# gk969/stm32-speech-recognition

Hardware: AMD Instinct MI355X
Metric: utterances/sec (256-frame, 100 templates) (higher is better)
Workload: dtype int32

## Files before the change

### stm32_speech_recognition_amd/csrc/k_mfcc.hip

```cpp
#include "sr_fft_dev.h"

#include <type_traits>

#ifndef SR_MEL_CHUNKED
#define SR_MEL_CHUNKED 1
#endif

namespace sr {

constexpr int kMfccWaves = 4;
constexpr int kFramesPerWave = 16, kFramesPerWaveMid = 4, kFramesPerWaveSmall = 1;
#ifndef SR_MAG_TAB_BINS
#define SR_MAG_TAB_BINS 8
#endif
constexpr int mfcc_tab_bins(int fpw) { return fpw == kFramesPerWave ? SR_MAG_TAB_BINS : 0; }
static_assert(SR_MAG_TAB_BINS == 0 || SR_MAG_TAB_BINS == 4 || SR_MAG_TAB_BINS == 8, "table bins per lane");
#ifndef SR_MFCC_PIPE
#define SR_MFCC_PIPE 1
#endif
#ifndef SR_MFCC_PIPE_PEEL
#define SR_MFCC_PIPE_PEEL 1
#endif
#ifndef SR_MFCC_PIPE_VMCNT
#define SR_MFCC_PIPE_VMCNT (SR_MFCC_PIPE_PEEL ? 3 : 0)
#endif
static_assert(SR_MFCC_PIPE_VMCNT == 0 || (SR_MFCC_PIPE_VMCNT == 3 && SR_MFCC_PIPE_PEEL), "younger loads counted by the wait");
constexpr bool mfcc_pipelined(int fpw) { return SR_MFCC_PIPE && mfcc_tab_bins(fpw) == 8; }
#ifndef SR_MFCC_TM_REGS
#define SR_MFCC_TM_REGS 1
#endif
#ifdef SR_INJECT_LDS_RACE
#undef SR_MFCC_TM_REGS
#define SR_MFCC_TM_REGS 0
#endif
constexpr bool mfcc_tm_regs(int fpw) { return SR_MFCC_TM_REGS && mfcc_pipelined(fpw); }
constexpr int kMelPad = kMel + 1;
__device__ __forceinline__ constexpr int mel_chunk_word(int j) { return 256 * ((j >> 2) & 1) + 4 * ((j >> 3) ^ (4 * ((j >> 2) & 1))) + (j & 3); }
#ifndef SR_MFCC_PREFIX_TID
#define SR_MFCC_PREFIX_TID 1
#endif
__device__ __forceinline__ constexpr int mel_prefix_word(int j)
{
#if SR_MFCC_PREFIX_TID
    return 64 * (j & 7) + (j >> 3);
#elif SR_MEL_CHUNKED
    return mel_chunk_word(j);
#else
    return j;
#endif
}
#pragma clang diagnostic push
#pragma clang diagnostic ignored "-Winline-asm"
__device__ __forceinline__ void mel_prefix_store(uint32_t base, const uint32_t (&pe)[8], const uint32_t (&po)[8])
{
    static_assert(kBins == 512, "the offsets below are written out for two halves of 512 words");
    asm volatile("s_mov_b32 m0, %16\n\ts_nop 0\n\t"
                 "ds_write_addtid_b32 %0\n\tds_write_addtid_b32 %1 offset:256\n\tds_write_addtid_b32 %2 offset:512\n\t"
                 "ds_write_addtid_b32 %3 offset:768\n\tds_write_addtid_b32 %4 offset:1024\n\tds_write_addtid_b32 %5 offset:1280\n\t"
                 "ds_write_addtid_b32 %6 offset:1536\n\tds_write_addtid_b32 %7 offset:1792\n\t"
                 "ds_write_addtid_b32 %8 offset:2048\n\tds_write_addtid_b32 %9 offset:2304\n\tds_write_addtid_b32 %10 offset:2560\n\t"
                 "ds_write_addtid_b32 %11 offset:2816\n\tds_write_addtid_b32 %12 offset:3072\n\tds_write_addtid_b32 %13 offset:3328\n\t"
                 "ds_write_addtid_b32 %14 offset:3584\n\tds_write_addtid_b32 %15 offset:3840"
                 :
                 : "v"(pe[0]), "v"(pe[1]), "v"(pe[2]), "v"(pe[3]), "v"(pe[4]), "v"(pe[5]), "v"(pe[6]), "v"(pe[7]), "v"(po[0]),
                   "v"(po[1]), "v"(po[2]), "v"(po[3]), "v"(po[4]), "v"(po[5]), "v"(po[6]), "v"(po[7]), "s"(base)
                 : "m0", "memory");
}
#pragma clang diagnostic pop
constexpr int mfcc_wave_lds_words(int fpw) { return kXchgWords + fpw * kMelPad + 64; }

template <typename Base>
struct MfccTabArgs : Base {
    const uint16_t *mag_q;
    uint32_t mag_table_off;
};
template <typename Base>
constexpr int mfcc_feat_kind<MfccTabArgs<Base>> = mfcc_feat_kind<Base>;
template <typename Base>
static MfccTabArgs<Base> mfcc_tab_args(const Base &b, const MfccMagTab &tab)
{
    MfccTabArgs<Base> r;
    static_cast<Base &>(r) = b;
    r.mag_q = tab.mag_q;
    r.mag_table_off = tab.mag_table_off;
    return r;
}

template <int kFPW, typename Args = MfccTabArgs<MfccArgs>>
__global__ void __launch_bounds__(64 * kMfccWaves, 4) k_mfcc(const Args a)
{
    constexpr int kFeat = mfcc_feat_kind<Args>;
    constexpr uint32_t kFeatW = (kFeat == SR_FEAT_FFT || kFeat == SR_FEAT_MAG) ? kBins : kMel;
    constexpr int kWaveLdsWords = mfcc_wave_lds_words(kFPW);
    constexpr int kTabBins = mfcc_tab_bins(kFPW);
    constexpr bool kPipe = mfcc_pipelined(kFPW);
    constexpr bool kTmRegs = mfcc_tm_regs(kFPW);
    extern __shared__ __attribute__((aligned(16))) uint32_t smem[];
    __shared__ uint32_t s_dctM[kCoef * kMelPad];
    __shared__ int s_dctS[kCoef * kMelPad];
    __shared__ u32x4 s_tw3[kTw3Row * 4], s_tw5[8 * 64];
    __shared__ u32x4 s_tm[4 * 64];
    const int lane = threadIdx.x & 63, w = __builtin_amdgcn_readfirstlane(threadIdx.x >> 6);
    uint32_t *buf = smem + w * kWaveLdsWords;
    uint32_t *xw = buf;
    uint32_t *powb = buf + kXchgWords, *moff = powb + kFPW * kMelPad;
    const uint32_t buf_lds = (uint32_t)(uintptr_t)(const __attribute__((address_space(3))) uint32_t *)buf;
    (void)buf_lds;

    for (int i = threadIdx.x; i < kCoef * kMel; i += blockDim.x) {
        const int c = a.t.dct[i], o = (i / kMel) * kMelPad + i % kMel;
        s_dctM[o] = (uint32_t)(((c < 0 ? -c : c) * 262144 + 99) / 100);
        s_dctS[o] = (c > 0) - (c < 0);
    }
    __syncthreads();

    LaneTw tw;
    load_lane_tw(a.t, lane, tw);
    real_leg_tw(tw);
    if (w == 0 && lane < 4) {
        const uint32_t *f = &tw.s3[0][0][0];
#pragma unroll
        for (int c = 0; c < 8; c++) s_tw3[lane * kTw3Row + c] = u32x4{f[4 * c], f[4 * c + 1], f[4 * c + 2], f[4 * c + 3]};
    }
    if (w == 1 % kMfccWaves) store_tw32(s_tw5, lane, tw.s5);
    u32x4 tm_r[4];
    if constexpr (kTmRegs) {
#pragma unroll
        for (int c = 0; c < 2; c++) {
            tm_r[c] = *(const u32x4 *)(a.t.tri_even_m + 8 * lane + 4 * c);
            tm_r[c + 2] = *(const u32x4 *)(a.t.tri_odd_m + 8 * lane + 4 * c);
        }
    }
#ifndef SR_INJECT_LDS_RACE
    if (!kTmRegs && w == 2 % kMfccWaves) {
#pragma unroll
        for (int c = 0; c < 2; c++) {
            s_tm[64 * c + lane] = *(const u32x4 *)(a.t.tri_even_m + 8 * lane + 4 * c);
            s_tm[64 * (c + 2) + lane] = *(const u32x4 *)(a.t.tri_odd_m + 8 * lane + 4 * c);
        }
    }
#endif
    __syncthreads();
#ifdef SR_INJECT_LDS_RACE
    if (w == 2 % kMfccWaves) {
#if SR_INJECT_LDS_RACE >= 2
        __builtin_amdgcn_s_sleep(127);
#endif
#pragma unroll
        for (int c = 0; c < 2; c++) {
            s_tm[64 * c + lane] = *(const u32x4 *)(a.t.tri_even_m + 8 * lane + 4 * c);
            s_tm[64 * (c + 2) + lane] = *(const u32x4 *)(a.t.tri_odd_m + 8 * lane + 4 * c);
        }
    }
#endif
    int hamm_m[3];
#pragma unroll
    for (int k = 0; k < 3; k++) hamm_m[k] = (lane + 64 * k < kFrameLen) ? hamm_fused_multiplier(a.t.hamm[lane + 64 * k]) : 0;
    int f_lo = 0, p_hi = 0, p_lo = 0, x_hi = 0, x_lo = 0;
    if (lane < kMel) {
        const int h = lane;
        f_lo = (h == 0) ? 0 : (int)a.t.tri_cen[h - 1];
        const int f_hi = (h == kMel - 1) ? kBins : (int)a.t.tri_cen[h + 1];
        const int ih = f_hi - 1, il = f_lo ? f_lo - 1 : 0, half = (h & 1) ? kBins : 0;
        p_hi = half + mel_prefix_word(ih), x_hi = (ih >> 3) > 0 ? (ih >> 3) - 1 : 0;
        p_lo = half + mel_prefix_word(il), x_lo = (il >> 3) > 0 ? (il >> 3) - 1 : 0;
    }
    const uint64_t mag_p = (uint64_t)a.mag_q;
    const u32x4 mag_rs = {(uint32_t)mag_p, (uint32_t)(mag_p >> 32) | (2u << 16), kMagTabEntries, 0x00027000u};
    const uint32_t tw_off = 32u * (uint32_t)lane;
#if SR_MEL_CHUNKED
    const int e_base = mel_chunk_word(lane);
    constexpr int kEs = 32, kEh = 128;
    const int c0 = mel_chunk_word(8 * lane), c1 = mel_chunk_word(8 * lane + 4);
#else
    const int e_base = lane;
    constexpr int kEs = 64, kEh = 256;
    const int c0 = 8 * lane, c1 = 8 * lane + 4;
#endif

    uint32_t item = blockIdx.x;
    uint32_t nx_nfrm = 0;
    int nx_mid = 0, nx_seg0 = 0;
    if (item < a.n_items) {
        const sr_vad_rec *rec = a.vad + item / a.tiles;
        nx_nfrm = rec->frm_num;
        nx_mid = (int)rec->atap.mid_val;
        nx_seg0 = rec->seg[0];
    }
    for (; item < a.n_items; item += gridDim.x) {
        const uint32_t b = item / a.tiles, tile = item - b * a.tiles;
        const uint32_t nfrm = nx_nfrm;
        const int mid = nx_mid, seg0 = nx_seg0;
        if (item + gridDim.x < a.n_items) {
            const sr_vad_rec *rec = a.vad + (item + gridDim.x) / a.tiles;
            nx_nfrm = rec->frm_num;
            nx_mid = (int)rec->atap.mid_val;
            nx_seg0 = rec->seg[0];
        }
        const uint16_t *row = a.pcm + (uint64_t)b * a.pcm_stride;
        int16_t *out = a.mfcc + (uint64_t)b * a.max_frames * kCoef;
        const uint32_t f0 = tile * (kMfccWaves * kFPW) + w * kFPW;
        uint32_t *frow = nullptr;
        if constexpr (kFeat != 0) frow = a.feat + (uint64_t)b * a.max_frames * kFeatW;
        uint32_t nf = 0;
        if (f0 < nfrm) nf = (nfrm - f0 < (uint32_t)kFPW) ? nfrm - f0 : (uint32_t)kFPW;

        uint32_t s_pp[3] = {0, 0, 0};
        if (nf) {
            const uint16_t *x = row + seg0 + (int)kHop * (int)f0;
#pragma unroll
            for (int k = 0; k < 3; k++) {
                const int i = lane + 64 * k;
                if (i < kFrameLen) s_pp[k] = *(const u32_align2 *)(x + i - 1);
            }
        }
        auto store_prefixes = [&](const uint32_t (&pe)[8], const uint32_t (&po)[8]) {
#if SR_MFCC_PREFIX_TID
            mel_prefix_store(buf_lds, pe, po);
#else
            *(uint4 *)(buf + c0) = make_uint4(pe[0], pe[1], pe[2], pe[3]);
            *(uint4 *)(buf + c1) = make_uint4(pe[4], pe[5], pe[6], pe[7]);
            *(uint4 *)(buf + kBins + c0) = make_uint4(po[0], po[1], po[2], po[3]);
            *(uint4 *)(buf + kBins + c1) = make_uint4(po[4], po[5], po[6], po[7]);
#endif
        };
        if constexpr (!kPipe)
        for (uint32_t fi = 0; fi < nf; fi++) {
#pragma unroll
            for (int k = 0; k < 3; k++) {
                const int i = lane + 64 * k;
                if (i < kFrameLen) k == 0 ? window_store<0>(xw, i, s_pp[k], mid, hamm_m[k]) : window_store<1>(xw, i, s_pp[k], mid, hamm_m[k]);
            }
            if (fi + 1 < nf) {
                const uint16_t *x = row + seg0 + (int)kHop * (int)(f0 + fi + 1);
#pragma unroll
                for (int k = 0; k < 3; k++) {
                    const int i = lane + 64 * k;
                    if (i < kFrameLen) s_pp[k] = *(const u32_align2 *)(x + i - 1);
                }
            }
            wave_sync();
            uint32_t v[4][4], u[4][4];
            fft_front_real160(xw, lane, tw, s_tw3, v);
            fft_exchange(buf, lane, v, u);
#pragma unroll
            for (int e4 = 0; e4 < 4; e4++) fft_pass4_dbl(u, e4, tw);
            wave_sync();
            uint32_t k5[4][4][2];
            load_tw32(s_tw5, lane, k5);
            uint32_t nn[8];
#pragma unroll
            for (int e3 = 0; e3 < 4; e3++) {
                bfly_pk_dbl<true, false, 0>(u[e3][0], u[e3][1], u[e3][2], u[e3][3], k5[e3][0][0], k5[e3][0][1], k5[e3][1][0],
                                            k5[e3][1][1], k5[e3][2][0], k5[e3][2][1], k5[e3][3][0], k5[e3][3][1]);
                if constexpr (kFeat == SR_FEAT_FFT) {
                    uint32_t *fr = frow + (f0 + fi) * kFeatW + lane + 64 * e3;
                    fr[0] = u[e3][0];
                    fr[256] = u[e3][1];
                }
                nn[2 * e3] = (uint32_t)sdot2z(u[e3][0], u[e3][0]);
                nn[2 * e3 + 1] = (uint32_t)sdot2z(u[e3][1], u[e3][1]);
            }
            const uint32_t nmax = max(max(max(max(nn[0], nn[1]), nn[2]), max(max(nn[3], nn[4]), nn[5])), max(nn[6], nn[7]));
#ifdef SR_TESTING
            const bool quiet = __builtin_expect(__builtin_amdgcn_ballot_w64(nmax > kMagSmallMax) == 0 && !a.mag_table_off, 1);
#else
            const bool quiet = __builtin_expect(__builtin_amdgcn_ballot_w64(nmax > kMagSmallMax) == 0, 1);
#endif
            u32x4 tw_e[2], tw_o[2];
            bool cheap = true;
            if (!quiet) {
#pragma unroll
                for (int c = 0; c < 2; c++) {
                    tw_e[c] = *(const u32x4 *)((const char *)a.t.tri_even32 + tw_off + 16 * c);
                    tw_o[c] = *(const u32x4 *)((const char *)a.t.tri_odd32 + tw_off + 16 * c);
                }
                cheap = __builtin_amdgcn_ballot_w64(nmax > a.mag_cheap_max) == 0;
            } else {
                asm volatile("" : "=v"(tw_e[0]), "=v"(tw_e[1]), "=v"(tw_o[0]), "=v"(tw_o[1]));
            }
            uint32_t *eb = buf + e_base;
            if (kTabBins > 0 && quiet) {
                uint32_t tq[8];
#pragma unroll
                for (int e3 = 0; e3 < 4; e3++) {
                    if constexpr (kTabBins == 8)
                        asm volatile("buffer_load_ushort %0, %1, %2, 0 idxen" : "=v"(tq[2 * e3]) : "v"(nn[2 * e3]), "s"(mag_rs));
                    asm volatile("buffer_load_ushort %0, %1, %2, 0 idxen" : "=v"(tq[2 * e3 + 1]) : "v"(nn[2 * e3 + 1]), "s"(mag_rs));
                }
                uint32_t q0s[4];
                if constexpr (kTabBins == 4) {
#pragma unroll
                    for (int e3 = 0; e3 < 4; e3++) q0s[e3] = cvt_u32(__builtin_amdgcn_sqrtf((float)(int)nn[2 * e3]) * 10.0f) << 2;
                }
                if constexpr (kTabBins == 8)
                    asm volatile("s_waitcnt vmcnt(0)" : "+v"(tq[0]), "+v"(tq[1]), "+v"(tq[2]), "+v"(tq[3]), "+v"(tq[4]), "+v"(tq[5]), "+v"(tq[6]), "+v"(tq[7]));
                else
                    asm volatile("s_waitcnt vmcnt(0)" : "+v"(tq[1]), "+v"(tq[3]), "+v"(tq[5]), "+v"(tq[7]));
#pragma unroll
                for (int e3 = 0; e3 < 4; e3++) {
                    uint32_t q0, q1 = tq[2 * e3 + 1];
                    if constexpr (kTabBins == 8) q0 = tq[2 * e3];
                    else q0 = q0s[e3];
                    if constexpr (kFeat == SR_FEAT_MAG) {
                        uint32_t *fr = frow + (f0 + fi) * kFeatW + lane + 64 * e3;
                        fr[0] = q0 >> 2;
                        fr[256] = q1 >> 2;
                    }
                    eb[kEs * e3] = umul24(q0, q0);
                    eb[kEs * e3 + kEh] = umul24(q1, q1);
                }
            } else if (cheap) {
#pragma unroll
                for (int e3 = 0; e3 < 4; e3++) {
                    const f32x2 m = f32x2{__builtin_amdgcn_sqrtf((float)(int)nn[2 * e3]), __builtin_amdgcn_sqrtf((float)(int)nn[2 * e3 + 1])} *
                                    f32x2{10.0f, 10.0f};
                    const uint32_t m0 = cvt_u32(m.x), m1 = cvt_u32(m.y);
                    if constexpr (kFeat == SR_FEAT_MAG) {
                        uint32_t *fr = frow + (f0 + fi) * kFeatW + lane + 64 * e3;
                        fr[0] = m0;
                        fr[256] = m1;
                    }
                    eb[kEs * e3] = umul24(m0, m0);
                    eb[kEs * e3 + kEh] = umul24(m1, m1);
                }
            } else {
#pragma unroll
                for (int e3 = 0; e3 < 4; e3++) {
                    const f32x2 m = sqrt_rn_int2(f32x2{(float)(int)nn[2 * e3], (float)(int)nn[2 * e3 + 1]}) * f32x2{10.0f, 10.0f};
                    const uint32_t m0 = cvt_u32(m.x), m1 = cvt_u32(m.y);
                    if constexpr (kFeat == SR_FEAT_MAG) {
                        uint32_t *fr = frow + (f0 + fi) * kFeatW + lane + 64 * e3;
                        fr[0] = m0;
                        fr[256] = m1;
                    }
                    eb[kEs * e3] = umul24(m0, m0);
                    eb[kEs * e3 + kEh] = umul24(m1, m1);
                }
            }
            wave_sync();
            uint32_t pe[8], po[8], xe, xo;
            {
                const uint4 q0 = *(const uint4 *)(buf + c0), q1 = *(const uint4 *)(buf + c1);
                const uint32_t e[8] = {q0.x, q0.y, q0.z, q0.w, q1.x, q1.y, q1.z, q1.w};
                uint32_t se = 0, so = 0;
                if (quiet) {
#pragma unroll
                    for (int c = 0; c < 2; c++) {
                        const u32x4 me = s_tm[64 * c + lane], mo = s_tm[64 * (c + 2) + lane];
#pragma unroll
                        for (int k = 0; k < 4; k++) {
                            const uint32_t es = kTabBins > 0 ? e[4 * c + k] : e[4 * c + k] << 4;
                            se += mel_term_fused(es, me[k]);
                            so += mel_term_fused(es, mo[k]);
                            pe[4 * c + k] = se;
                            po[4 * c + k] = so;
                        }
                    }
                } else {
#pragma unroll
                    for (int c = 0; c < 2; c++) {
#pragma unroll
                        for (int k = 0; k < 4; k++) {
                            se += e[4 * c + k] * tw_e[c][k] / 100u;
                            so += e[4 * c + k] * tw_o[c][k] / 100u;
                            pe[4 * c + k] = se;
                            po[4 * c + k] = so;
                        }
                    }
                }
                xe = wave_scan_incl(se);
                xo = wave_scan_incl(so);
            }
            store_prefixes(pe, po);
            buf[2 * kBins + lane] = xe;
            moff[lane] = xo;
            wave_sync();
            if (lane < kMel) {
                const uint32_t *X = (lane & 1) ? moff : buf + 2 * kBins;
                const uint32_t hi = buf[p_hi] + X[x_hi], lo = f_lo ? buf[p_lo] + X[x_lo] : 0u;
                powb[fi * kMelPad + lane] = hi - lo;
                if constexpr (kFeat == SR_FEAT_MEL) frow[(f0 + fi) * kFeatW + lane] = hi - lo;
            }
            wave_sync();
        } else {
            uint32_t mq[8] = {0, 0, 0, 0, 0, 0, 0, 0};
            bool pq = true;
            auto window = [&]() {
#pragma unroll
                for (int k = 0; k < 3; k++) {
                    const int i = lane + 64 * k;
                    if (i < kFrameLen) k == 0 ? window_store<0>(xw, i, s_pp[k], mid, hamm_m[k]) : window_store<1>(xw, i, s_pp[k], mid, hamm_m[k]);
                }
            };
            auto request = [&](uint32_t f) {
                const uint16_t *x = row + seg0 + (int)kHop * (int)(f0 + f);
#pragma unroll
                for (int k = 0; k < 3; k++) {
                    const int i = lane + 64 * k;
                    if (i < kFrameLen) s_pp[k] = *(const u32_align2 *)(x + i - 1);
                }
            };
            auto middle = [&](uint32_t fi, uint32_t (&v)[4][4], bool more) {
                uint32_t u[4][4];
                fft_exchange(buf, lane, v, u);
#pragma unroll
                for (int e4 = 0; e4 < 4; e4++) fft_pass4_dbl(u, e4, tw);
                wave_sync();
                uint32_t k5[4][4][2];
                load_tw32(s_tw5, lane, k5);
                uint32_t nn[8];
#pragma unroll
                for (int e3 = 0; e3 < 4; e3++) {
                    bfly_pk_dbl<true, false, 0>(u[e3][0], u[e3][1], u[e3][2], u[e3][3], k5[e3][0][0], k5[e3][0][1], k5[e3][1][0],
                                                k5[e3][1][1], k5[e3][2][0], k5[e3][2][1], k5[e3][3][0], k5[e3][3][1]);
                    if constexpr (kFeat == SR_FEAT_FFT) {
                        uint32_t *fr = frow + (f0 + fi) * kFeatW + lane + 64 * e3;
                        fr[0] = u[e3][0];
                        fr[256] = u[e3][1];
                    }
                    nn[2 * e3] = (uint32_t)sdot2z(u[e3][0], u[e3][0]);
                    nn[2 * e3 + 1] = (uint32_t)sdot2z(u[e3][1], u[e3][1]);
                }
                const uint32_t nmax = max(max(max(max(nn[0], nn[1]), nn[2]), max(max(nn[3], nn[4]), nn[5])), max(nn[6], nn[7]));
                if (more) {
                    wave_sync();
                    window();
                }
#ifdef SR_TESTING
                const bool quiet = __builtin_expect(__builtin_amdgcn_ballot_w64(nmax > kMagSmallMax) == 0 && !a.mag_table_off, 1);
#else
                const bool quiet = __builtin_expect(__builtin_amdgcn_ballot_w64(nmax > kMagSmallMax) == 0, 1);
#endif
                if (quiet) {
#pragma unroll
                    for (int k = 0; k < 8; k++) asm volatile("buffer_load_ushort %0, %1, %2, 0 idxen" : "=v"(mq[k]) : "v"(nn[k]), "s"(mag_rs));
                } else if (__builtin_amdgcn_ballot_w64(nmax > a.mag_cheap_max) == 0) {
#pragma unroll
                    for (int e3 = 0; e3 < 4; e3++) {
                        const f32x2 m = f32x2{__builtin_amdgcn_sqrtf((float)(int)nn[2 * e3]), __builtin_amdgcn_sqrtf((float)(int)nn[2 * e3 + 1])} *
                                        f32x2{10.0f, 10.0f};
                        mq[2 * e3] = cvt_u32(m.x);
                        mq[2 * e3 + 1] = cvt_u32(m.y);
                    }
                } else {
#pragma unroll
                    for (int e3 = 0; e3 < 4; e3++) {
                        const f32x2 m = sqrt_rn_int2(f32x2{(float)(int)nn[2 * e3], (float)(int)nn[2 * e3 + 1]}) * f32x2{10.0f, 10.0f};
                        mq[2 * e3] = cvt_u32(m.x);
                        mq[2 * e3 + 1] = cvt_u32(m.y);
                    }
                }
                pq = quiet;
                if (fi + 2 < nf) request(fi + 2);
            };
            auto back_end = [&](uint32_t r, auto young) {
                wave_sync();
                auto energies = [&]() {
                    uint32_t *eb = buf + e_base;
#pragma unroll
                    for (int e3 = 0; e3 < 4; e3++) {
                        const uint32_t q0 = mq[2 * e3], q1 = mq[2 * e3 + 1];
                        if constexpr (kFeat == SR_FEAT_MAG) {
                            uint32_t *fr = frow + (f0 + r) * kFeatW + lane + 64 * e3;
                            const uint32_t sh = pq ? 2u : 0u;
                            fr[0] = q0 >> sh;
                            fr[256] = q1 >> sh;
                        }
                        eb[kEs * e3] = umul24(q0, q0);
                        eb[kEs * e3 + kEh] = umul24(q1, q1);
                    }
                    wave_sync();
                };
                uint32_t pe[8], po[8], se = 0, so = 0;
                if (pq) {
                    if constexpr (decltype(young)::value)
                        asm volatile("s_waitcnt vmcnt(3)" : "+v"(mq[0]), "+v"(mq[1]), "+v"(mq[2]), "+v"(mq[3]), "+v"(mq[4]), "+v"(mq[5]), "+v"(mq[6]), "+v"(mq[7]));
                    else
                        asm volatile("s_waitcnt vmcnt(0)" : "+v"(mq[0]), "+v"(mq[1]), "+v"(mq[2]), "+v"(mq[3]), "+v"(mq[4]), "+v"(mq[5]), "+v"(mq[6]), "+v"(mq[7]));
                    energies();
                    const uint4 q0 = *(const uint4 *)(buf + c0), q1 = *(const uint4 *)(buf + c1);
                    const uint32_t e[8] = {q0.x, q0.y, q0.z, q0.w, q1.x, q1.y, q1.z, q1.w};
#pragma unroll
                    for (int c = 0; c < 2; c++) {
                        u32x4 me, mo;
                        if constexpr (kTmRegs) me = tm_r[c], mo = tm_r[c + 2];
                        else me = s_tm[64 * c + lane], mo = s_tm[64 * (c + 2) + lane];
#pragma unroll
                        for (int k = 0; k < 4; k++) {
                            se += mel_term_fused(e[4 * c + k], me[k]);
                            so += mel_term_fused(e[4 * c + k], mo[k]);
                            pe[4 * c + k] = se;
                            po[4 * c + k] = so;
                        }
                    }
                } else {
                    u32x4 tw_e[2], tw_o[2];
                    uint32_t off = tw_off;
                    asm("" : "+v"(off));
#pragma unroll
                    for (int c = 0; c < 2; c++) {
                        tw_e[c] = *(const u32x4 *)((const char *)a.t.tri_even32 + off + 16 * c);
                        tw_o[c] = *(const u32x4 *)((const char *)a.t.tri_odd32 + off + 16 * c);
                    }
                    energies();
                    const uint4 q0 = *(const uint4 *)(buf + c0), q1 = *(const uint4 *)(buf + c1);
                    const uint32_t e[8] = {q0.x, q0.y, q0.z, q0.w, q1.x, q1.y, q1.z, q1.w};
#pragma unroll
                    for (int c = 0; c < 2; c++) {
#pragma unroll
                        for (int k = 0; k < 4; k++) {
                            se += e[4 * c + k] * tw_e[c][k] / 100u;
                            so += e[4 * c + k] * tw_o[c][k] / 100u;
                            pe[4 * c + k] = se;
                            po[4 * c + k] = so;
                        }
                    }
                }
                const uint32_t xe = wave_scan_incl(se), xo = wave_scan_incl(so);
                store_prefixes(pe, po);
                buf[2 * kBins + lane] = xe;
                moff[lane] = xo;
                wave_sync();
                if (lane < kMel) {
// ... 198 lines not shown
```

### stm32_speech_recognition_amd/csrc/k_mfcc_gen.hip

```cpp
#include "sr_fft_dev.h"

namespace sr {

constexpr int kGenWaves = 4;
constexpr int kGenMaxMel = 64;
constexpr int kGenWaveWords = kNfft + kNfft + kXchgWords + kBins + kGenMaxMel;

struct GenTw {
    LaneTw tw;
    uint32_t k2[3][2];
};
__device__ __forceinline__ void load_gen_tw(const DevTables &t, int lane, GenTw &g)
{
    load_lane_tw(t, lane, g.tw);
    load_tw3(t, 0, lane & 3, g.k2);
}
__device__ __forceinline__ void fft_real_half(const uint32_t *__restrict__ in, uint32_t *__restrict__ out, uint32_t *buf, int lane,
                                              const GenTw &g)
{
    for (int m = 0; m < 4; m++) {
        const int idx = lane + 64 * m, r = bitrev8(idx);
        int ar = sext_lo(in[r]), br = sext_lo(in[r + 512]), cr = sext_lo(in[r + 256]), dr = sext_lo(in[r + 768]);
        int ai = 0, bi = 0, ci = 0, di = 0;
        r4_combine<0>(ar, ai, br, bi, cr, ci, dr, di);
        buf[xaddr(4 * idx + 0)] = pack16(ar, ai);
        buf[xaddr(4 * idx + 1)] = pack16(br, bi);
        buf[xaddr(4 * idx + 2)] = pack16(cr, ci);
        buf[xaddr(4 * idx + 3)] = pack16(di, dr);
    }
    wave_sync();
    const LaneTw &tw = g.tw;
    const int d0 = lane & 3, d3 = (lane >> 2) & 3, d4 = lane >> 4;
    uint32_t v[4][4], u[4][4];
#pragma unroll
    for (int d1 = 0; d1 < 4; d1++)
#pragma unroll
        for (int d2 = 0; d2 < 4; d2++) v[d1][d2] = buf[xaddr(d0 + 4 * d1 + 16 * d2 + 64 * d3 + 256 * d4)];
    wave_sync();
#pragma unroll
    for (int d2 = 0; d2 < 4; d2++)
        bfly(v[0][d2], v[1][d2], v[2][d2], v[3][d2], g.k2[0][0], g.k2[0][1], g.k2[1][0], g.k2[1][1], g.k2[2][0], g.k2[2][1]);
#pragma unroll
    for (int d1 = 0; d1 < 4; d1++)
        bfly_pk<false>(v[d1][0], v[d1][1], v[d1][2], v[d1][3], tw.s3[d1][0][0], tw.s3[d1][0][1], tw.s3[d1][1][0], tw.s3[d1][1][1],
                       tw.s3[d1][2][0], tw.s3[d1][2][1], tw.s3[d1][3][0], tw.s3[d1][3][1]);
    fft_exchange(buf, lane, v, u);
#pragma unroll
    for (int e4 = 0; e4 < 4; e4++)
        bfly_pk<false>(u[0][e4], u[1][e4], u[2][e4], u[3][e4], tw.s4[0][0], tw.s4[0][1], tw.s4[1][0], tw.s4[1][1], tw.s4[2][0],
                       tw.s4[2][1], tw.s4[3][0], tw.s4[3][1]);
#pragma unroll
    for (int e3 = 0; e3 < 4; e3++) {
        bfly_pk<true>(u[e3][0], u[e3][1], u[e3][2], u[e3][3], tw.s5[e3][0][0], tw.s5[e3][0][1], tw.s5[e3][1][0], tw.s5[e3][1][1],
                      tw.s5[e3][2][0], tw.s5[e3][2][1], tw.s5[e3][3][0], tw.s5[e3][3][1]);
        out[lane + 64 * e3] = u[e3][0];
        out[lane + 64 * e3 + 256] = u[e3][1];
    }
}

template <typename Args = MfccArgs>
__global__ void __launch_bounds__(64 * kGenWaves) k_mfcc_gen(const Args a)
{
    constexpr int kFeat = mfcc_feat_kind<Args>;
    extern __shared__ __attribute__((aligned(16))) uint32_t smem[];
    const int lane = threadIdx.x & 63, w = threadIdx.x >> 6;
    uint32_t *fin = smem + (size_t)w * kGenWaveWords, *fout = fin + kNfft, *buf = fout + kNfft, *en = buf + kXchgWords,
             *pw = en + kBins;
// ... 133 lines not shown
```

### stm32_speech_recognition_amd/csrc/sr_fft_dev.h

```cpp
#pragma once
#include <type_traits>

#include "sr_dev.h"

namespace sr {

__device__ __forceinline__ void cxmul(uint32_t y, uint32_t ka, uint32_t kb, int &re, int &im)
{
    re = sdot2z(y, ka);
    im = sdot2z(y, kb);
}

template <int S>
__device__ __forceinline__ void r4_combine(int &ar, int &ai, int &br, int &bi, int &cr, int &ci, int &dr, int &di)
{
    int tr = cr + dr, ti = ci + di;
    dr = cr - dr;
    di = ci - di;
    cr = tr;
    ci = ti;
    ar >>= 2;
    ai >>= 2;
    ar += br >> (2 + S);
    ai += bi >> (2 + S);
    br = ar - (br >> (1 + S));
    bi = ai - (bi >> (1 + S));
    ar += cr >> (2 + S);
    ai += ci >> (2 + S);
    cr = ar - (cr >> (1 + S));
    ci = ai - (ci >> (1 + S));
    br += di >> (2 + S);
    bi -= dr >> (2 + S);
    di = br - (di >> (1 + S));
    dr = bi + (dr >> (1 + S));
}

constexpr uint32_t kPkPlusMinus = 0xFFFF0001u;
constexpr uint32_t kPkMinusPlus = 0x0001FFFFu;

template <bool HALF, bool HAS_B, bool CD_SAME = false, bool A_SHIFTED = false>
__device__ __forceinline__ void r4_packed(uint32_t x0_in, int br, int bi, int sr, int si, int tr, int ti, uint32_t &x0,
                                          uint32_t &x1, uint32_t &x2, uint32_t &x3)
{
    const uint32_t a = A_SHIFTED ? x0_in : pk_ashr(x0_in, 2);
    uint32_t A1 = a, B1 = a;
    if (HAS_B) {
        A1 = pk_add(a, pk_hi16(br, bi));
        B1 = pk_sub(A1, pk_s15(br, bi));
    }
    const uint32_t hC = pk_hi16(sr, si);
    x0 = pk_add(A1, hC);
    x1 = CD_SAME ? pk_mad_swap(hC, kPkPlusMinus, B1) : pk_mad(pk_hi16(ti, tr), kPkPlusMinus, B1);
    if (!HALF) {
        const uint32_t pC = pk_s15(sr, si);
        x2 = pk_sub(x0, pC);
        x3 = CD_SAME ? pk_mad_swap(pC, kPkMinusPlus, x1) : pk_mad(pk_s15(ti, tr), kPkMinusPlus, x1);
// ... 43 lines not shown
    if (DBL_CD) {
        pC = pk_hi16(sr, si);
        hC = pk_ashr(pC, 1);
    } else {
        hC = pk_hi16(sr, si);
        if (!HALF) pC = pk_s15(sr, si);
    }
    x0 = madd(hC, P, P, kStraight, A1);
    uint32_t pD = 0, hD;
    if (CD_SAME) {
        pD = pC;
        hD = hC;
    } else if (DBL_CD) {
        pD = pk_hi16(ti, tr);
        hD = pk_ashr(pD, 1);
    } else {
        hD = pk_hi16(ti, tr);
        if (!HALF) pD = pk_s15(ti, tr);
    }
    x1 = madd(hD, P, N, kSwapC, B1);
    if (!HALF) {
        x2 = madd(pC, N, N, kStraight, x0);
        x3 = madd(pD, N, P, kSwapC, x1);
    }
}

template <bool HALF, bool DBL_CD, int OUT>
__device__ __forceinline__ void bfly_pk_dbl(uint32_t &x0, uint32_t &x1, uint32_t &x2, uint32_t &x3, uint32_t k1a,
                                            uint32_t k1b, uint32_t k2a, uint32_t k2b, uint32_t k3a, uint32_t k3b,
                                            uint32_t k3na, uint32_t k3nb, uint32_t mul = 0)
{
    int br, bi, cr, ci;
    cxmul(x2, k2a, k2b, cr, ci);
    cxmul(x1, k1a, k1b, br, bi);
    const int sr = sdot2a(x3, k3a, cr), si = sdot2a(x3, k3b, ci);
    const int tr = sdot2a(x3, k3na, cr), ti = sdot2a(x3, k3nb, ci);
    uint32_t a = pk_ashr(x0, 2);
    if (OUT == 1) a = pk_add(a, a);
    if (OUT == 2) a = pk_mul_lo_lo(a, mul);
    r4_packed_dbl<HALF, true, false, DBL_CD, OUT>(a, mul, br, bi, sr, si, tr, ti, x0, x1, x2, x3);
}

__device__ __forceinline__ uint32_t pk_neg(uint32_t w) { return pk_sub(0u, w); }

__device__ __forceinline__ void bfly(uint32_t &x0, uint32_t &x1, uint32_t &x2, uint32_t &x3, uint32_t k1a, uint32_t k1b,
                                     uint32_t k2a, uint32_t k2b, uint32_t k3a, uint32_t k3b)
{
    bfly_pk<false>(x0, x1, x2, x3, k1a, k1b, k2a, k2b, k3a, k3b, pk_neg(k3a), pk_neg(k3b));
}

__device__ __forceinline__ int rev2(int d) { return ((d & 1) << 1) | (d >> 1); }

__device__ __forceinline__ int xaddr(int j) { return j + ((j >> 6) << 2); }
constexpr int kXchgWords = 1024 + 4 * 16;

struct LaneTw {
    uint32_t s2[2][2];
    uint32_t s3[4][4][2];
    uint32_t s4[4][2];
    uint32_t s5[4][4][2];
};

__device__ __forceinline__ void load_tw3(const DevTables &t, int base, int b, uint32_t (&k)[3][2])
{
    const int e = base + 3 * b;
    k[0][0] = t.tw_a[e + 2];
    k[0][1] = t.tw_b[e + 2];
    k[1][0] = t.tw_a[e + 1];
    k[1][1] = t.tw_b[e + 1];
    k[2][0] = t.tw_a[e + 0];
    k[2][1] = t.tw_b[e + 0];
}

__device__ __forceinline__ void load_tw4(const DevTables &t, int base, int b, uint32_t (&k)[4][2])
{
    uint32_t k3[3][2];
    load_tw3(t, base, b, k3);
#pragma unroll
    for (int e = 0; e < 3; e++) {
        k[e][0] = k3[e][0];
        k[e][1] = k3[e][1];
    }
    k[3][0] = pk_sub(0u, k3[2][0]);
    k[3][1] = pk_sub(0u, k3[2][1]);
}

__device__ __forceinline__ void load_lane_tw(const DevTables &t, int lane, LaneTw &tw)
{
    const int d0 = lane & 3;
    {
        uint32_t k[3][2];
        load_tw3(t, 0, d0, k);
        tw.s2[0][0] = k[0][0];
        tw.s2[0][1] = k[0][1];
        tw.s2[1][0] = k[1][0];
        tw.s2[1][1] = k[1][1];
    }
#pragma unroll
    for (int d1 = 0; d1 < 4; d1++) load_tw4(t, 12, d0 + 4 * d1, tw.s3[d1]);
    load_tw4(t, 60, lane, tw.s4);
#pragma unroll
    for (int d3 = 0; d3 < 4; d3++) load_tw4(t, 252, lane + 64 * d3, tw.s5[d3]);
}

__device__ __forceinline__ void store_tw32(u32x4 *lds, int lane, const uint32_t (&k)[4][4][2])
{
    const uint32_t *f = &k[0][0][0];
#pragma unroll
    for (int c = 0; c < 8; c++) lds[c * 64 + lane] = u32x4{f[4 * c], f[4 * c + 1], f[4 * c + 2], f[4 * c + 3]};
}
__device__ __forceinline__ void load_tw32(const u32x4 *lds, int lane, uint32_t (&k)[4][4][2])
{
    uint32_t *f = &k[0][0][0];
#pragma unroll
    for (int c = 0; c < 8; c++) {
        const u32x4 q = lds[c * 64 + lane];
        f[4 * c] = q.x;
        f[4 * c + 1] = q.y;
        f[4 * c + 2] = q.z;
        f[4 * c + 3] = q.w;
    }
}
constexpr int kTw3Row = 9;
__device__ __forceinline__ void load_tw32_d0(const u32x4 *lds, int d0, uint32_t (&k)[4][4][2])
{
    uint32_t *f = &k[0][0][0];
#pragma unroll
    for (int c = 0; c < 8; c++) {
        const u32x4 q = lds[d0 * kTw3Row + c];
        f[4 * c] = q.x;
        f[4 * c + 1] = q.y;
        f[4 * c + 2] = q.z;
        f[4 * c + 3] = q.w;
    }
}

constexpr uint32_t kPkOneTwo = 0x00020001u;
template <int K>
__device__ __forceinline__ void window_store(uint32_t *xw, int i, uint32_t prev_cur, int mid, int hm)
{
    if (K == 0) {
        xw[i] = pk_mul_lo_dup(window_sample<4>(prev_cur, mid, hm), kPkOneTwo);
    } else {
        const uint32_t y = window_sample<2>(prev_cur, mid, hm);
        xw[i] = y;
        ((uint16_t *)(xw + i))[1] = (uint16_t)y;
    }
}
__device__ __forceinline__ void real_leg_tw(LaneTw &tw)
{
#pragma unroll
    for (int l = 0; l < 2; l++)
#pragma unroll
        for (int w = 0; w < 2; w++) tw.s2[l][w] = __builtin_amdgcn_perm(0u, tw.s2[l][w], 0x01000100u);
}
__device__ __forceinline__ void fft_front_real160(const uint32_t *xw, int lane, const LaneTw &tw, const u32x4 *tw3_lds,
                                                  uint32_t (&v)[4][4])
{
    const int d3 = (lane >> 2) & 3, d4 = lane >> 4;
    const int base = rev2(d4) + 4 * rev2(d3);
    uint32_t y[10];
    y[0] = *(const uint16_t *)(xw + base);
#pragma unroll
    for (int m = 1; m < 4; m++) y[m] = ((const uint16_t *)(xw + base + 16 * m))[1];
#pragma unroll
    for (int m = 4; m < 10; m++) y[m] = xw[base + 16 * m];
#pragma unroll
    for (int m = 0; m < 4; m++) asm("" : "+v"(y[m]));
#pragma unroll
    for (int d2 = 0; d2 < 4; d2++) {
        const int r2 = ((d2 & 1) << 1) | (d2 >> 1);
        uint32_t x0 = y[r2];
        uint32_t x2 = y[4 + r2];
        uint32_t x1 = (d2 == 0) ? y[8] : (d2 == 2) ? y[9] : 0u;
        uint32_t x3 = 0u;
        int cr, ci;
        cxmul(x2, tw.s2[1][0], tw.s2[1][1], cr, ci);
        (void)x3;
        if (d2 == 0) {
            int br, bi;
            cxmul(x1, tw.s2[0][0], tw.s2[0][1], br, bi);
            r4_packed_dbl<false, true, true, true, 0>(x0, 0u, br, bi, cr, ci, cr, ci, v[0][d2], v[1][d2], v[2][d2], v[3][d2]);
        } else if (d2 == 2) {
            int br, bi;
            cxmul(x1, tw.s2[0][0], tw.s2[0][1], br, bi);
            r4_packed_dbl<false, true, true, true, 1>(x0, 0u, br, bi, cr, ci, cr, ci, v[0][d2], v[1][d2], v[2][d2], v[3][d2]);
        } else {
            r4_packed_dbl<false, false, true, true, 1>(x0, 0u, 0, 0, cr, ci, cr, ci, v[0][d2], v[1][d2], v[2][d2], v[3][d2]);
        }
    }
    uint32_t k3[4][4][2];
    load_tw32_d0(tw3_lds, lane & 3, k3);
    const uint32_t mul = d3 ? kPkTwo : kPkPlusMinus;
#pragma unroll
    for (int d1 = 0; d1 < 4; d1++)
        bfly_pk_dbl<false, true, 2>(v[d1][0], v[d1][1], v[d1][2], v[d1][3], k3[d1][0][0], k3[d1][0][1], k3[d1][1][0], k3[d1][1][1],
                                    k3[d1][2][0], k3[d1][2][1], k3[d1][3][0], k3[d1][3][1], mul);
}

__device__ __forceinline__ void fft_exchange(uint32_t *buf, int lane, const uint32_t (&v)[4][4], uint32_t (&u)[4][4])
{
    const int d0 = lane & 3, d3 = (lane >> 2) & 3, d4 = lane >> 4;
    const int jw = d0 + 64 * d3 + 256 * d4;
#pragma unroll
    for (int d1 = 0; d1 < 4; d1++)
#pragma unroll
        for (int d2 = 0; d2 < 4; d2++) buf[xaddr(jw + 4 * d1 + 16 * d2)] = v[d1][d2];
    wave_sync();
#pragma unroll
    for (int e3 = 0; e3 < 4; e3++)
#pragma unroll
        for (int e4 = 0; e4 < 4; e4++) u[e3][e4] = buf[xaddr(lane + 64 * e3 + 256 * e4)];
}

__device__ __forceinline__ void fft_pass4_dbl(uint32_t (&u)[4][4], int e4, const LaneTw &tw)
{
    if (e4 == 1)
        bfly_pk_dbl<false, true, 1>(u[0][e4], u[1][e4], u[2][e4], u[3][e4], tw.s4[0][0], tw.s4[0][1], tw.s4[1][0], tw.s4[1][1],
                                    tw.s4[2][0], tw.s4[2][1], tw.s4[3][0], tw.s4[3][1]);
    else
        bfly_pk_dbl<false, true, 0>(u[0][e4], u[1][e4], u[2][e4], u[3][e4], tw.s4[0][0], tw.s4[0][1], tw.s4[1][0], tw.s4[1][1],
                                    tw.s4[2][0], tw.s4[2][1], tw.s4[3][0], tw.s4[3][1]);
}

__device__ __forceinline__ int bitrev8(int v) { return (int)(__brev((uint32_t)v) >> 24); }

__device__ inline void fft_full_wave(const uint32_t *__restrict__ in, uint32_t *__restrict__ out, uint32_t *buf, int lane,
                              const DevTables &t)
{
    for (int m = 0; m < 4; m++) {
        const int idx = lane + 64 * m, r = bitrev8(idx);
        const uint32_t wa = in[r], wc = in[r + 256], wb = in[r + 512], wd = in[r + 768];
        int ar = sext_lo(wa), ai = sext_hi(wa), br = sext_lo(wb), bi = sext_hi(wb);
        int cr = sext_lo(wc), ci = sext_hi(wc), dr = sext_lo(wd), di = sext_hi(wd);
        r4_combine<0>(ar, ai, br, bi, cr, ci, dr, di);
        buf[xaddr(4 * idx + 0)] = pack16(ar, ai);
        buf[xaddr(4 * idx + 1)] = pack16(br, bi);
        buf[xaddr(4 * idx + 2)] = pack16(cr, ci);
        buf[xaddr(4 * idx + 3)] = pack16(di, dr);
    }
    wave_sync();
    LaneTw tw;
    load_lane_tw(t, lane, tw);
    uint32_t k2[3][2];
    load_tw3(t, 0, lane & 3, k2);
    const int d0 = lane & 3, d3 = (lane >> 2) & 3, d4 = lane >> 4;
    uint32_t v[4][4], u[4][4];
#pragma unroll
    for (int d1 = 0; d1 < 4; d1++)
#pragma unroll
        for (int d2 = 0; d2 < 4; d2++) v[d1][d2] = buf[xaddr(d0 + 4 * d1 + 16 * d2 + 64 * d3 + 256 * d4)];
    wave_sync();
#pragma unroll
    for (int d2 = 0; d2 < 4; d2++)
        bfly(v[0][d2], v[1][d2], v[2][d2], v[3][d2], k2[0][0], k2[0][1], k2[1][0], k2[1][1], k2[2][0], k2[2][1]);
#pragma unroll
    for (int d1 = 0; d1 < 4; d1++)
        bfly(v[d1][0], v[d1][1], v[d1][2], v[d1][3], tw.s3[d1][0][0], tw.s3[d1][0][1], tw.s3[d1][1][0],
             tw.s3[d1][1][1], tw.s3[d1][2][0], tw.s3[d1][2][1]);
    fft_exchange(buf, lane, v, u);
#pragma unroll
    for (int e4 = 0; e4 < 4; e4++)
        bfly(u[0][e4], u[1][e4], u[2][e4], u[3][e4], tw.s4[0][0], tw.s4[0][1], tw.s4[1][0], tw.s4[1][1], tw.s4[2][0],
             tw.s4[2][1]);
#pragma unroll
    for (int e3 = 0; e3 < 4; e3++) {
        bfly(u[e3][0], u[e3][1], u[e3][2], u[e3][3], tw.s5[e3][0][0], tw.s5[e3][0][1], tw.s5[e3][1][0],
             tw.s5[e3][1][1], tw.s5[e3][2][0], tw.s5[e3][2][1]);
#pragma unroll
        for (int e4 = 0; e4 < 4; e4++) out[lane + 64 * e3 + 256 * e4] = u[e3][e4];
    }
}

}
```

Before: 3.390 million.

## Use ds_write_addtid stores with padded planes for FFT exchange and mel energies

Reassigns FFT front lanes so d0 becomes the high lane bits. The exchange and the power-spectrum energies are now written with ds_write_addtid_b32 into padded per-plane LDS images and read back with 128-bit loads. A new layout header holds compile-time checks for the consistency of the mapping and for bank-conflict freedom of the b128 reads. The aim is fewer LDS instructions and fewer address computations in the per-frame exchange and energy stages, at the cost of inline asm that sets m0 and hardcoded offsets.

```diff
diff --git a/stm32_speech_recognition_amd/csrc/k_mfcc.hip b/stm32_speech_recognition_amd/csrc/k_mfcc.hip
--- a/stm32_speech_recognition_amd/csrc/k_mfcc.hip
+++ b/stm32_speech_recognition_amd/csrc/k_mfcc.hip
@@ -1,10 +1,6 @@
 #include "sr_fft_dev.h"
 
 #include <type_traits>
-
-#ifndef SR_MEL_CHUNKED
-#define SR_MEL_CHUNKED 1
-#endif
 
 namespace sr {
 
@@ -35,20 +31,7 @@
 #endif
 constexpr bool mfcc_tm_regs(int fpw) { return SR_MFCC_TM_REGS && mfcc_pipelined(fpw); }
 constexpr int kMelPad = kMel + 1;
-__device__ __forceinline__ constexpr int mel_chunk_word(int j) { return 256 * ((j >> 2) & 1) + 4 * ((j >> 3) ^ (4 * ((j >> 2) & 1))) + (j & 3); }
-#ifndef SR_MFCC_PREFIX_TID
-#define SR_MFCC_PREFIX_TID 1
-#endif
-__device__ __forceinline__ constexpr int mel_prefix_word(int j)
-{
-#if SR_MFCC_PREFIX_TID
-    return 64 * (j & 7) + (j >> 3);
-#elif SR_MEL_CHUNKED
-    return mel_chunk_word(j);
-#else
-    return j;
-#endif
-}
+__device__ __forceinline__ constexpr int mel_prefix_word(int j) { return 64 * (j & 7) + (j >> 3); }
 #pragma clang diagnostic push
 #pragma clang diagnostic ignored "-Winline-asm"
 __device__ __forceinline__ void mel_prefix_store(uint32_t base, const uint32_t (&pe)[8], const uint32_t (&po)[8])
@@ -64,6 +47,19 @@
                  :
                  : "v"(pe[0]), "v"(pe[1]), "v"(pe[2]), "v"(pe[3]), "v"(pe[4]), "v"(pe[5]), "v"(pe[6]), "v"(pe[7]), "v"(po[0]),
                    "v"(po[1]), "v"(po[2]), "v"(po[3]), "v"(po[4]), "v"(po[5]), "v"(po[6]), "v"(po[7]), "s"(base)
+                 : "m0", "memory");
+}
+__device__ __forceinline__ void mel_energy_store(uint32_t base, const uint32_t (&en)[8])
+{
+    static_assert(4 * energy_plane(1) == 256 && 4 * energy_plane(2) == 528 && 4 * energy_plane(3) == 784 && 4 * energy_plane(4) == 1040 &&
+                      4 * energy_plane(5) == 1296 && 4 * energy_plane(6) == 1568 && 4 * energy_plane(7) == 1824 && kBins == kEnergyBins,
+                  "the offsets below are written out for these plane bases");
+    asm volatile("s_mov_b32 m0, %8\n\ts_nop 0\n\t"
+                 "ds_write_addtid_b32 %0\n\tds_write_addtid_b32 %1 offset:256\n\tds_write_addtid_b32 %2 offset:528\n\t"
+                 "ds_write_addtid_b32 %3 offset:784\n\tds_write_addtid_b32 %4 offset:1040\n\tds_write_addtid_b32 %5 offset:1296\n\t"
+                 "ds_write_addtid_b32 %6 offset:1568\n\tds_write_addtid_b32 %7 offset:1824"
+                 :
+                 : "v"(en[0]), "v"(en[2]), "v"(en[4]), "v"(en[6]), "v"(en[1]), "v"(en[3]), "v"(en[5]), "v"(en[7]), "s"(base)
                  : "m0", "memory");
 }
 #pragma clang diagnostic pop
@@ -115,12 +111,13 @@
     __syncthreads();
 
     LaneTw tw;
-    load_lane_tw(a.t, lane, tw);
+    load_lane_tw(a.t, lane, lane >> 4, tw);
     real_leg_tw(tw);
-    if (w == 0 && lane < 4) {
+    if (w == 0 && (lane & 15) == 0) {
         const uint32_t *f = &tw.s3[0][0][0];
-#pragma unroll
-        for (int c = 0; c < 8; c++) s_tw3[lane * kTw3Row + c] = u32x4{f[4 * c], f[4 * c + 1], f[4 * c + 2], f[4 * c + 3]};
+        const int d0 = lane >> 4;
+#pragma unroll
+        for (int c = 0; c < 8; c++) s_tw3[d0 * kTw3Row + c] = u32x4{f[4 * c], f[4 * c + 1], f[4 * c + 2], f[4 * c + 3]};
     }
     if (w == 1 % kMfccWaves) store_tw32(s_tw5, lane, tw.s5);
     u32x4 tm_r[4];
@@ -168,15 +165,7 @@
     const uint64_t mag_p = (uint64_t)a.mag_q;
     const u32x4 mag_rs = {(uint32_t)mag_p, (uint32_t)(mag_p >> 32) | (2u << 16), kMagTabEntries, 0x00027000u};
     const uint32_t tw_off = 32u * (uint32_t)lane;
-#if SR_MEL_CHUNKED
-    const int e_base = mel_chunk_word(lane);
-    constexpr int kEs = 32, kEh = 128;
-    const int c0 = mel_chunk_word(8 * lane), c1 = mel_chunk_word(8 * lane + 4);
-#else
-    const int e_base = lane;
-    constexpr int kEs = 64, kEh = 256;
-    const int c0 = 8 * lane, c1 = 8 * lane + 4;
-#endif
+    const int c0 = energy_read_base(lane), c1 = c0 + 4;
 
     uint32_t item = blockIdx.x;
     uint32_t nx_nfrm = 0;
@@ -214,16 +203,9 @@
                 if (i < kFrameLen) s_pp[k] = *(const u32_align2 *)(x + i - 1);
             }
         }
-        auto store_prefixes = [&](const uint32_t (&pe)[8], const uint32_t (&po)[8]) {
-#if SR_MFCC_PREFIX_TID
-            mel_prefix_store(buf_lds, pe, po);
-#else
-            *(uint4 *)(buf + c0) = make_uint4(pe[0], pe[1], pe[2], pe[3]);
-            *(uint4 *)(buf + c1) = make_uint4(pe[4], pe[5], pe[6], pe[7]);
-            *(uint4 *)(buf + kBins + c0) = make_uint4(po[0], po[1], po[2], po[3]);
-            *(uint4 *)(buf + kBins + c1) = make_uint4(po[4], po[5], po[6], po[7]);
-#endif
-        };
+        auto store_prefixes = [&](const uint32_t (&pe)[8], const uint32_t (&po)[8]) { mel_prefix_store(buf_lds, pe, po); };
+        auto store_energies = [&](const uint32_t (&en)[8]) { mel_energy_store(buf_lds, en); };
+        auto exchange = [&](const uint32_t (&v)[4][4], uint32_t (&u)[4][4]) { fft_exchange_tid(buf, buf_lds, lane, v, u); };
         if constexpr (!kPipe)
         for (uint32_t fi = 0; fi < nf; fi++) {
 #pragma unroll
@@ -242,7 +224,7 @@
             wave_sync();
             uint32_t v[4][4], u[4][4];
             fft_front_real160(xw, lane, tw, s_tw3, v);
-            fft_exchange(buf, lane, v, u);
+            exchange(v, u);
 #pragma unroll
             for (int e4 = 0; e4 < 4; e4++) fft_pass4_dbl(u, e4, tw);
             wave_sync();
@@ -279,7 +261,7 @@
             } else {
                 asm volatile("" : "=v"(tw_e[0]), "=v"(tw_e[1]), "=v"(tw_o[0]), "=v"(tw_o[1]));
             }
-            uint32_t *eb = buf + e_base;
+            uint32_t en[8];
             if (kTabBins > 0 && quiet) {
                 uint32_t tq[8];
 #pragma unroll
@@ -307,8 +289,8 @@
                         fr[0] = q0 >> 2;
                         fr[256] = q1 >> 2;
                     }
-                    eb[kEs * e3] = umul24(q0, q0);
-                    eb[kEs * e3 + kEh] = umul24(q1, q1);
+                    en[2 * e3] = umul24(q0, q0);
+                    en[2 * e3 + 1] = umul24(q1, q1);
                 }
             } else if (cheap) {
 #pragma unroll
@@ -321,8 +303,8 @@
                         fr[0] = m0;
                         fr[256] = m1;
                     }
-                    eb[kEs * e3] = umul24(m0, m0);
-                    eb[kEs * e3 + kEh] = umul24(m1, m1);
+                    en[2 * e3] = umul24(m0, m0);
+                    en[2 * e3 + 1] = umul24(m1, m1);
                 }
             } else {
 #pragma unroll
@@ -334,10 +316,11 @@
                         fr[0] = m0;
                         fr[256] = m1;
                     }
-                    eb[kEs * e3] = umul24(m0, m0);
-                    eb[kEs * e3 + kEh] = umul24(m1, m1);
-                }
-            }
+                    en[2 * e3] = umul24(m0, m0);
+                    en[2 * e3 + 1] = umul24(m1, m1);
+                }
+            }
+            store_energies(en);
             wave_sync();
             uint32_t pe[8], po[8], xe, xo;
             {
@@ -403,7 +386,7 @@
             };
             auto middle = [&](uint32_t fi, uint32_t (&v)[4][4], bool more) {
                 uint32_t u[4][4];
-                fft_exchange(buf, lane, v, u);
+                exchange(v, u);
 #pragma unroll
                 for (int e4 = 0; e4 < 4; e4++) fft_pass4_dbl(u, e4, tw);
                 wave_sync();
@@ -457,7 +440,7 @@
             auto back_end = [&](uint32_t r, auto young) {
                 wave_sync();
                 auto energies = [&]() {
-                    uint32_t *eb = buf + e_base;
+                    uint32_t en[8];
 #pragma unroll
                     for (int e3 = 0; e3 < 4; e3++) {
                         const uint32_t q0 = mq[2 * e3], q1 = mq[2 * e3 + 1];
@@ -467,9 +450,10 @@
                             fr[0] = q0 >> sh;
                             fr[256] = q1 >> sh;
                         }
-                        eb[kEs * e3] = umul24(q0, q0);
-                        eb[kEs * e3 + kEh] = umul24(q1, q1);
-                    }
+                        en[2 * e3] = umul24(q0, q0);
+                        en[2 * e3 + 1] = umul24(q1, q1);
+                    }
+                    store_energies(en);
                     wave_sync();
                 };
                 uint32_t pe[8], po[8], se = 0, so = 0;
diff --git a/stm32_speech_recognition_amd/csrc/k_mfcc_gen.hip b/stm32_speech_recognition_amd/csrc/k_mfcc_gen.hip
--- a/stm32_speech_recognition_amd/csrc/k_mfcc_gen.hip
+++ b/stm32_speech_recognition_amd/csrc/k_mfcc_gen.hip
@@ -12,7 +12,7 @@
 };
 __device__ __forceinline__ void load_gen_tw(const DevTables &t, int lane, GenTw &g)
 {
-    load_lane_tw(t, lane, g.tw);
+    load_lane_tw(t, lane, lane & 3, g.tw);
     load_tw3(t, 0, lane & 3, g.k2);
 }
 __device__ __forceinline__ void fft_real_half(const uint32_t *__restrict__ in, uint32_t *__restrict__ out, uint32_t *buf, int lane,
diff --git a/stm32_speech_recognition_amd/csrc/sr_fft_dev.h b/stm32_speech_recognition_amd/csrc/sr_fft_dev.h
--- a/stm32_speech_recognition_amd/csrc/sr_fft_dev.h
+++ b/stm32_speech_recognition_amd/csrc/sr_fft_dev.h
@@ -2,6 +2,7 @@
 #include <type_traits>
 
 #include "sr_dev.h"
+#include "sr_fft_layout.h"
 
 namespace sr {
 
@@ -151,7 +152,6 @@
 __device__ __forceinline__ int rev2(int d) { return ((d & 1) << 1) | (d >> 1); }
 
 __device__ __forceinline__ int xaddr(int j) { return j + ((j >> 6) << 2); }
-constexpr int kXchgWords = 1024 + 4 * 16;
 
 struct LaneTw {
     uint32_t s2[2][2];
@@ -184,9 +184,8 @@
     k[3][1] = pk_sub(0u, k3[2][1]);
 }
 
-__device__ __forceinline__ void load_lane_tw(const DevTables &t, int lane, LaneTw &tw)
-{
-    const int d0 = lane & 3;
+__device__ __forceinline__ void load_lane_tw(const DevTables &t, int lane, int d0, LaneTw &tw)
+{
     {
         uint32_t k[3][2];
         load_tw3(t, 0, d0, k);
@@ -256,7 +255,7 @@
 __device__ __forceinline__ void fft_front_real160(const uint32_t *xw, int lane, const LaneTw &tw, const u32x4 *tw3_lds,
                                                   uint32_t (&v)[4][4])
 {
-    const int d3 = (lane >> 2) & 3, d4 = lane >> 4;
+    const int d0 = lane >> 4, d3 = lane & 3, d4 = (lane >> 2) & 3;
     const int base = rev2(d4) + 4 * rev2(d3);
     uint32_t y[10];
     y[0] = *(const uint16_t *)(xw + base);
@@ -289,7 +288,7 @@
         }
     }
     uint32_t k3[4][4][2];
-    load_tw32_d0(tw3_lds, lane & 3, k3);
+    load_tw32_d0(tw3_lds, d0, k3);
     const uint32_t mul = d3 ? kPkTwo : kPkPlusMinus;
 #pragma unroll
     for (int d1 = 0; d1 < 4; d1++)
@@ -311,6 +310,35 @@
 #pragma unroll
         for (int e4 = 0; e4 < 4; e4++) u[e3][e4] = buf[xaddr(lane + 64 * e3 + 256 * e4)];
 }
+
+#pragma clang diagnostic push
+#pragma clang diagnostic ignored "-Winline-asm"
+__device__ __forceinline__ void fft_exchange_tid(const uint32_t *buf, uint32_t base, int lane, const uint32_t (&v)[4][4], uint32_t (&u)[4][4])
+{
+    static_assert(4 * kXchgPlane == 272 && xchg_plane(1, 0) == 1 && xchg_plane(0, 1) == 4, "the offsets below are written out for planes d1 + 4 d2 of 68 words");
+    asm volatile("s_mov_b32 m0, %16\n\ts_nop 0\n\t"
+                 "ds_write_addtid_b32 %0\n\tds_write_addtid_b32 %1 offset:272\n\tds_write_addtid_b32 %2 offset:544\n\t"
+                 "ds_write_addtid_b32 %3 offset:816\n\tds_write_addtid_b32 %4 offset:1088\n\tds_write_addtid_b32 %5 offset:1360\n\t"
+                 "ds_write_addtid_b32 %6 offset:1632\n\tds_write_addtid_b32 %7 offset:1904\n\t"
+                 "ds_write_addtid_b32 %8 offset:2176\n\tds_write_addtid_b32 %9 offset:2448\n\tds_write_addtid_b32 %10 offset:2720\n\t"
+                 "ds_write_addtid_b32 %11 offset:2992\n\tds_write_addtid_b32 %12 offset:3264\n\tds_write_addtid_b32 %13 offset:3536\n\t"
+                 "ds_write_addtid_b32 %14 offset:3808\n\tds_write_addtid_b32 %15 offset:4080"
+                 :
+                 : "v"(v[0][0]), "v"(v[1][0]), "v"(v[2][0]), "v"(v[3][0]), "v"(v[0][1]), "v"(v[1][1]), "v"(v[2][1]), "v"(v[3][1]),
+                   "v"(v[0][2]), "v"(v[1][2]), "v"(v[2][2]), "v"(v[3][2]), "v"(v[0][3]), "v"(v[1][3]), "v"(v[2][3]), "v"(v[3][3]), "s"(base)
+                 : "m0", "memory");
+    wave_sync();
+    const u32x4 *rd = (const u32x4 *)(buf + xchg_read_base(lane));
+#pragma unroll
+    for (int e4 = 0; e4 < 4; e4++) {
+        const u32x4 q = rd[e4];
+        u[0][e4] = q.x;
+        u[1][e4] = q.y;
+        u[2][e4] = q.z;
+        u[3][e4] = q.w;
+    }
+}
+#pragma clang diagnostic pop
 
 __device__ __forceinline__ void fft_pass4_dbl(uint32_t (&u)[4][4], int e4, const LaneTw &tw)
 {
@@ -340,7 +368,7 @@
     }
     wave_sync();
     LaneTw tw;
-    load_lane_tw(t, lane, tw);
+    load_lane_tw(t, lane, lane & 3, tw);
     uint32_t k2[3][2];
     load_tw3(t, 0, lane & 3, k2);
     const int d0 = lane & 3, d3 = (lane >> 2) & 3, d4 = lane >> 4;
diff --git a/stm32_speech_recognition_amd/csrc/sr_fft_layout.h b/stm32_speech_recognition_amd/csrc/sr_fft_layout.h
--- /dev/null
+++ b/stm32_speech_recognition_amd/csrc/sr_fft_layout.h
@@ -0,0 +1,94 @@
+#pragma once
+
+namespace sr {
+
+constexpr int kXchgWords = 1024 + 4 * 16;
+
+constexpr int kXchgPlane = 68;
+constexpr int xchg_front_lane(int d0, int d3, int d4) { return d3 + 4 * d4 + 16 * d0; }
+constexpr int xchg_front_elem(int lane, int d1, int d2) { return (lane >> 4) + 4 * d1 + 16 * d2 + 64 * (lane & 3) + 256 * ((lane >> 2) & 3); }
+constexpr int xchg_plane(int d1, int d2) { return d1 + 4 * d2; }
+constexpr int xchg_store_word(int lane, int d1, int d2) { return kXchgPlane * xchg_plane(d1, d2) + lane; }
+constexpr int xchg_read_base(int rl, int plane_stride = kXchgPlane) { return plane_stride * (rl >> 2) + 16 * (rl & 3); }
+constexpr int xchg_read_word(int rl, int e3, int e4) { return xchg_read_base(rl) + e3 + 4 * e4; }
+constexpr int kXchgImageWords = xchg_store_word(63, 3, 3) + 1;
+
+constexpr int kEnergyBins = 512;
+constexpr int energy_plane(int q) { return 64 * q + 4 * ((q + 2) >> 2); }
+constexpr int energy_store_word(int lane, int e3, int half) { return energy_plane(e3 + 4 * half) + lane; }
+constexpr int energy_word(int bin) { return energy_plane(bin >> 6) + (bin & 63); }
+constexpr int energy_read_base(int l, int plane_stride = 0) { return (plane_stride ? plane_stride * (l >> 3) : energy_plane(l >> 3)) + 8 * (l & 7); }
+constexpr int kEnergyImageWords = energy_word(kEnergyBins - 1) + 1;
+
+constexpr int b128_group(int lane)
+{
+    const int l = lane & 31;
+    return ((l < 4 || (l >= 12 && l < 16) || (l >= 20 && l < 28)) ? 0 : 1) + 2 * (lane >> 5);
+}
+template <class F>
+constexpr int b128_extra_cycles(F word_of_lane)
+{
+    int extra = 0;
+    for (int g = 0; g < 4; g++) {
+        int first[16] = {}, lanes = 0, worst = 1;
+        for (int lane = 0; lane < 64; lane++)
+            if (b128_group(lane) == g) first[lanes++] = word_of_lane(lane);
+        for (int bank = 0; bank < 64; bank++) {
+            int seen[16] = {}, n = 0;
+            for (int k = 0; k < lanes; k++) {
+                const int a = first[k];
+                if (((bank - a) & 63) >= 4) continue;
+                bool known = false;
+                for (int i = 0; i < n; i++) known = known || seen[i] == a;
+                if (!known) seen[n++] = a;
+            }
+            if (n > worst) worst = n;
+        }
+        extra += worst - 1;
+    }
+    return extra;
+}
+constexpr int xchg_read_extra_cycles(int e4, int plane_stride = kXchgPlane)
+{
+    return b128_extra_cycles([=](int lane) { return xchg_read_base(lane, plane_stride) + 4 * e4; });
+}
+constexpr int energy_read_extra_cycles(int second, int plane_stride = 0)
+{
+    return b128_extra_cycles([=](int lane) { return energy_read_base(lane, plane_stride) + 4 * second; });
+}
+
+constexpr bool xchg_image_consistent()
+{
+    bool elem[1024] = {}, word[kXchgWords] = {};
+    for (int lane = 0; lane < 64; lane++)
+        for (int d1 = 0; d1 < 4; d1++)
+            for (int d2 = 0; d2 < 4; d2++) {
+                const int j = xchg_front_elem(lane, d1, d2), at = xchg_store_word(lane, d1, d2);
+                if (j < 0 || j >= 1024 || at < 0 || at >= kXchgWords || elem[j] || word[at]) return false;
+                elem[j] = word[at] = true;
+                if (xchg_read_word(j & 63, (j >> 6) & 3, j >> 8) != at) return false;
+                if (xchg_front_lane(j & 3, (j >> 6) & 3, j >> 8) != lane) return false;
+            }
+    return true;
+}
+constexpr bool energy_image_consistent()
+{
+    bool word[kEnergyImageWords] = {};
+    for (int b = 0; b < kEnergyBins; b++) {
+        const int at = energy_store_word(b & 63, (b >> 6) & 3, b >> 8);
+        if (at < 0 || at >= kEnergyImageWords || word[at]) return false;
+        word[at] = true;
+        if (energy_word(b) != at || energy_read_base(b >> 3) + (b & 7) != at) return false;
+    }
+    return true;
+}
+static_assert(xchg_image_consistent() && kXchgImageWords <= kXchgWords, "exchange image");
+static_assert(energy_image_consistent() && kEnergyImageWords <= kXchgWords, "energies image");
+static_assert(xchg_read_base(63) % 4 == 0 && kXchgPlane % 4 == 0 && energy_read_base(63) % 4 == 0 && energy_plane(7) % 4 == 0, "16-byte reads are aligned");
+static_assert(xchg_read_extra_cycles(0) == 0 && xchg_read_extra_cycles(1) == 0 && xchg_read_extra_cycles(2) == 0 && xchg_read_extra_cycles(3) == 0,
+              "exchange reads are conflict-free");
+static_assert(energy_read_extra_cycles(0) == 0 && energy_read_extra_cycles(1) == 0, "energy reads are conflict-free");
+static_assert(xchg_read_extra_cycles(0, 64) == 12 && xchg_read_extra_cycles(0, 72) == 4 && energy_read_extra_cycles(0, 64) > 0,
+              "the model sees the conflicts of the plain strides");
+
+}
```

Result: faster. 3.438 million, median of 6 (+1.4%).
